# VikParuchuri/surya

Hardware: AMD Instinct MI355X
Metric: text-lines/sec recognised (whole node) (higher is better)
Workload: dtype bf16; 1 GPU; RecognitionPredictor device loop, 256 ragged 64x{128..512} crops/GPU, batch 256, max_tokens=48, REC-FULL synthetic weights (conditioned recipe, seed 0), tiles resident in HBM; parallelism=1 GPU, weights=conditioned

## Files before the change

surya_amd/csrc/common.h:

```cpp
#pragma once
#include <hip/hip_runtime.h>
#include <cstdlib>
#include <stdint.h>
#include <stdio.h>
#include <type_traits>

#include "../../include/surya_amd.h"

namespace sa {

typedef unsigned short bf16_t;
typedef __attribute__((ext_vector_type(4))) float f32x4;
typedef __attribute__((ext_vector_type(16))) float f32x16;
typedef __attribute__((ext_vector_type(8))) __bf16 bf16x8;
typedef unsigned int u32x4 __attribute__((ext_vector_type(4)));


#define SA_HIP(expr)                                                                                   \
    do {                                                                                               \
        hipError_t _e = (expr);                                                                        \
        if (_e != hipSuccess) {                                                                        \
            fprintf(stderr, "[surya_amd] %s:%d %s -> %s\n", __FILE__, __LINE__, #expr, hipGetErrorString(_e)); \
            return (int)_e;                                                                            \
        }                                                                                              \
// ... 163 lines not shown
    e8 = e + 127;
    return mx_pack4(ldexpf(v[0], -e), ldexpf(v[1], -e), ldexpf(v[2], -e), ldexpf(v[3], -e));
}

__device__ __forceinline__ float wave_sum(float v) {
#pragma unroll
    for (int o = 32; o > 0; o >>= 1) v += __shfl_xor(v, o, 64);
    return v;
}
__device__ __forceinline__ float wave_max(float v) {
#pragma unroll
    for (int o = 32; o > 0; o >>= 1) v = fmaxf(v, __shfl_xor(v, o, 64));
    return v;
}

__device__ __forceinline__ float silu_f(float x) { return x / (1.0f + __expf(-x)); }
template <typename TI>
__device__ __forceinline__ float silu_epi(float x) {
    if constexpr (sizeof(TI) == 2) return x * __builtin_amdgcn_rcpf(1.0f + __expf(-x));
    else return silu_f(x);
}
__device__ __forceinline__ float gelu_erf_f(float x) { return 0.5f * x * (1.0f + erff(x * 0.70710678118654752440f)); }
template <typename TI>
__device__ __forceinline__ float gelu_epi(float x) {
    if constexpr (std::is_same<TI, fp16_t>::value) {
        const float xr = Ty<fp16_t>::rnd(x);
        const float z = fabsf(xr) * 0.70710678118654752440f;
        const float t = __builtin_amdgcn_rcpf(fmaf(0.5f, z, 1.0f));
        float p = fmaf(t, 0.17087277f, -0.82215223f);
        p = fmaf(t, p, 1.48851587f);
        p = fmaf(t, p, -1.13520398f);
        p = fmaf(t, p, 0.27886807f);
        p = fmaf(t, p, -0.18628806f);
        p = fmaf(t, p, 0.09678418f);
        p = fmaf(t, p, 0.37409196f);
        p = fmaf(t, p, 1.00002368f);
        p = fmaf(t, p, -1.26551223f);
        const float e = t * __expf(fmaf(-z, z, p));
        return 0.5f * xr * (xr < 0.f ? e : 2.0f - e);
    } else if constexpr (sizeof(TI) == 2) {
        const float z = fabsf(x) * 0.70710678118654752440f;
        const float t = __builtin_amdgcn_rcpf(fmaf(0.3275911f, z, 1.0f));
        const float poly = t * fmaf(t, fmaf(t, fmaf(t, fmaf(t, 1.061405429f, -1.453152027f), 1.421413741f), -0.284496736f), 0.254829592f);
        const float erfc_abs = poly * __expf(-z * z);
        return 0.5f * x * (x < 0.f ? erfc_abs : 2.0f - erfc_abs);
    } else {
        return gelu_erf_f(x);
    }
}
__device__ __forceinline__ float gelu_tanh_f(float x) { return 0.5f * x * (1.0f + tanhf(0.7978845608028654f * (x + 0.044715f * x * x * x))); }
__device__ __forceinline__ float sigmoid_f(float x) { return 1.0f / (1.0f + __expf(-x)); }
__device__ __forceinline__ float hardswish_f(float x) {
    float t;
    asm("v_fma_f32 %0, %1, %2, 0.5 clamp" : "=v"(t) : "v"(x), "s"(1.0f / 6.0f));
    return x * t;
}
typedef float f32x2_hs __attribute__((ext_vector_type(2)));
__device__ __forceinline__ f32x2_hs hardswish_pk(f32x2_hs x) {
    f32x2_hs t;
    const f32x2_hs c = {1.0f / 6.0f, 1.0f / 6.0f};
    asm("v_pk_fma_f32 %0, %1, %2, 0.5 op_sel_hi:[1,0,0] clamp" : "=v"(t) : "v"(x), "s"(c));
    return x * t;
}

struct Tuning {
    int graph = 0;
    int split_target = 256;
    int split_min_kt = 4;
    int split_max = 8;
    int bigtile = 3;
    int bigtile_any = 0;
    int big_m_split = -1;
    int big_m_gateup = -1;
    int mx_big_m_split = -1;
    int mx_big_m_gateup = -1;
    int gateup_ring = 2;
    int dring = 1;
    int dring_min_kt = 0;
    int conv_persist = 3;
    int dwconv_pipe = 2;
    int conv_lean = 1;
    int bigtile_ratio_pct = 0;
    int bigtile_min_k = 0;
    int glds = 2;
    int dattn = 4;
    int rnorm = 2;
    int ghead = 2;
    int fuse_embed = 1;
    int kvprefetch = 0;
    int lmhead = 1;
    int dattn_db = 0;
    int lay_ln = 1;
    int det_head_blk = 1;
    int det_fuse = 1023;
    int det_up4 = 1;
    int fmb_chunk = 64;
    int persist = 1;
    int ocrerr_cls_only = 1;
};
inline Tuning& tuning() { static Tuning t; return t; }
inline int& tuning_epoch() { static int e = 0; return e; }

inline void poison_arena(void* p, size_t bytes) {
    static const bool on = [] { const char* e = getenv("SURYA_AMD_POISON"); return e && e[0] == '1'; }();
    if (on) { (void)hipMemset(p, 0xFF, bytes); (void)hipDeviceSynchronize(); }
}

struct AttrOnce {
    size_t granted[64] = {};
    template <typename F> void ensure(F kern, size_t lds) {
        int dev = 0;
        (void)hipGetDevice(&dev);
        size_t& g = granted[dev & 63];
        if (lds > g || g == 0) {
            (void)hipFuncSetAttribute(reinterpret_cast<const void*>(kern), hipFuncAttributeMaxDynamicSharedMemorySize, (int)lds);
            g = lds > g ? lds : g;
            if (g == 0) g = 1;
        }
    }
};

constexpr int SA_ALT_NONE = 0x7fffffff;
__device__ __forceinline__ bool alt_after(float v, int c, float pv, int pc) { return (v < pv) | ((v == pv) & (c > pc)); }
__device__ __forceinline__ bool alt_before(float v, int c, float bv, int bc) { return (v > bv) | ((v == bv) & (c < bc)); }
__device__ __forceinline__ float2 alt_next(const float2* cand, int n, float pv, int pc) {
    float cb = -INFINITY;
    int ci = SA_ALT_NONE;
    for (int k = 0; k < n; ++k) {
        const float v = cand[k].x;
        const int cc = __float_as_int(cand[k].y);
        const bool take = (v > -INFINITY) & alt_after(v, cc, pv, pc) & alt_before(v, cc, cb, ci);
        cb = take ? v : cb;
        ci = take ? cc : ci;
    }
    return make_float2(cb, __int_as_float(ci));
}

static inline int cdiv(int a, int b) { return (a + b - 1) / b; }
static inline long cdivl(long a, long b) { return (a + b - 1) / b; }

}
```

surya_amd/csrc/gemm.h:

```cpp
#pragma once
#include <algorithm>
#include <cstdlib>
#include <type_traits>

#include "common.h"
#include "fastdiv.h"

namespace sa {

enum GemmEpi { EPI_BIAS = 0, EPI_RESIDUAL = 1, EPI_GELU = 2, EPI_SWIGLU = 3, EPI_HARDSWISH = 4, EPI_RELU = 5, EPI_ARGMAX = 6, EPI_ROPE = 7,
               EPI_GEGLU = 8 ,
               EPI_ARGMAX_MASK = 9 ,
               EPI_TOPK = 10 ,
               EPI_FORCED = 11  };
constexpr bool epi_is_argmax(int epi) { return epi == EPI_ARGMAX || epi == EPI_ARGMAX_MASK || epi == EPI_TOPK || epi == EPI_FORCED; }
constexpr bool epi_is_masked(int epi) { return epi == EPI_ARGMAX_MASK || epi == EPI_TOPK; }

struct TokenMask {
    const uint32_t* table = nullptr;
    const int* slot_mask = nullptr;
    const int* row_slot = nullptr;
    int words = 0;
    __device__ __forceinline__ int id_of(int m, int M) const {
        const int gm = min(m, M - 1);
        return slot_mask[row_slot ? row_slot[gm] : gm];
    }
    __device__ __forceinline__ uint32_t word_of(int mid, int w) const {
        const uint32_t v = table[(long)max(mid, 0) * words + min(w, words - 1)];
        return mid < 0 ? 0xffffffffu : v;
    }
    __device__ __forceinline__ int id_or_none(int m, int M) const { return table ? id_of(m, M) : -1; }
    __device__ __forceinline__ uint32_t word_or_all(int mid, int w) const {
        return mid < 0 ? 0xffffffffu : table[(long)mid * words + min(w, words - 1)];
    }
};

struct ForcedCols {
    const int* table = nullptr;
    const int* cursor = nullptr;
    const int* row_slot = nullptr;
    int stride = 0;
    float* flogit = nullptr;
    __device__ __forceinline__ int col_of(int m, int M, int N) const {
        if (m >= M) return -1;
        const int slot = row_slot ? row_slot[m] : m;
        const int cur = cursor ? cursor[slot] : 0;
        const int c = table[(long)slot * stride + min(max(cur, 0), stride - 1)];
        return (cur >= 0 && cur < stride && c < N) ? c : -1;
    }
};

template <typename TI, typename TO>
struct GemmArgs {
    const TI* X; long ldx;
    const TI* W; long ldw;
    TO* C; long ldc;
    const TI* bias;
    const TO* R; long ldr;
    int M, N, K;
    int splitk = 1;
    float* part = nullptr;
    int swz_m = 0, swz_n = 0;
    int mgroup = 0;
    float4* amax = nullptr;
    mutable int bn_used = 0;
    TokenMask tmask;
    float2* alt = nullptr;
    ForcedCols forced;
    const float2* rope = nullptr;
    int rope_cols = 0, rope_D = 0;
    const TI* conv_in = nullptr;
    const TI* conv_zero = nullptr;
    int cH = 0, cW = 0, cCin = 0, cHo = 0, cWo = 0, cKW = 0, cStride = 0, cPad = 0, cTaps = 0;
    int conv_lean = 1;
    FastDiv fd_hw, fd_wo;
    unsigned cv_m1 = 0, cv_m2 = 0;
    int cv_rowskip = 0;
#ifndef SA_P8_TIMING
#define SA_P8_TIMING 0
#endif
#if SA_P8_TIMING
    long long* dbg = nullptr;
#endif
};

template <typename TI> struct Mfma;
template <> struct Mfma<bf16_t> {
    __device__ static __forceinline__ void run(f32x16& acc, const u32x4& w, const u32x4& x) { acc = H16<bf16_t>::mfma(w, x, acc); }
};
// ... 1407 lines not shown
#if SA_P8_TIMING
        ++dbg_tile;
#endif
        if (!have_next) return;
        tile_m = nt_m; tile_n = nt_n;
    }
#undef SP_STAMP
#undef SP_PHASE
#undef SP_VM
#undef SP_MMA
#undef SP_RW
#undef SP_RX
#undef SP_REQX
#undef SP_REQW
#undef SP_REQ
}
#undef SA_COMPUTE
#undef SA_COMPUTE_FULL
#undef SA_COMPUTE_LEAN
#undef SA_FRAGS
#undef SA_MFMAS

struct GemmProfiler {
    static constexpr int NCFG = 4, POOL = 8192;
    static constexpr int NCFG_ALL = 6;
    bool enabled = false;
    hipEvent_t ev[2 * POOL];
    bool have_events = false;
    int n = 0;
    int cfg_of[POOL];
    double flops_of[POOL], bytes_of[POOL], slab_of[POOL];
    void start() {
        if (!have_events) {
            for (int i = 0; i < 2 * POOL; ++i) (void)hipEventCreate(&ev[i]);
            have_events = true;
        }
        n = 0; enabled = true;
    }
};
inline GemmProfiler& gemm_profiler() { static GemmProfiler p; return p; }
inline int gemm_cfg_id(int BM, int BN) { return (BM >= 128 && BN >= 128) ? 0 : (BM == 256 ? 1 : 2); }

template <typename TI, typename TO, int BM, int BN, int WM, int WN, int EPI, bool SPLIT = false, int GLDS = 0, bool CONV = false, int WAUX = 0>
static inline int launch_gemm_cfg(const GemmArgs<TI, TO>& a, hipStream_t s) {
    int tiles = SPLIT ? cdiv(cdiv(a.N, BN) * a.splitk, 8) * 8 * cdiv(a.M, BM) : cdiv(a.M, BM) * cdiv(a.N, BN);
    a.bn_used = BN;
    GemmArgs<TI, TO> aa = a;
    if (!SPLIT && !a.mgroup && BM >= 128 && BN >= 128) {
        const int tm = cdiv(a.M, BM), tn = cdiv(a.N, BN);
        constexpr int GRP = ((BM + BN) * 128 * (GLDS > 2 && GLDS != 8 ? GLDS : 2) > 80 * 1024) ? 32 : 64;
        if (tm * tn >= 8 * GRP) {
            aa.swz_n = cdiv(tn, cdiv(tn, 8));
            aa.swz_m = std::max(1, GRP / aa.swz_n);
            tiles = cdiv(tm * tn, 8 * GRP) * 8 * GRP;
        }
    }
    if (!SPLIT && aa.mgroup) tiles = cdiv(cdiv(a.N, BN), 8) * 8 * cdiv(a.M, BM);
    constexpr size_t out_w = ((EPI == EPI_SWIGLU || EPI == EPI_GEGLU) && !SPLIT) ? BN / 2 : BN;
    constexpr size_t out_bytes = (size_t)BM * out_w * (SPLIT ? sizeof(float) : sizeof(TO));
    constexpr size_t stage_bytes = (size_t)(BM + BN) * 128 * (GLDS > 2 && GLDS != 8 ? GLDS : 2);
    constexpr bool argmax_direct = epi_is_argmax(EPI) && ((size_t)BM * BN * 4 > 160 * 1024);
    constexpr size_t lds = (argmax_direct || stage_bytes > out_bytes) ? stage_bytes : out_bytes;
    auto kern = gemm_nt_kernel<TI, TO, BM, BN, WM, WN, EPI, SPLIT, GLDS, CONV, WAUX>;
    static AttrOnce attr;
    attr.ensure(kern, lds);
    GemmProfiler& pf = gemm_profiler();
    const bool prof = pf.enabled && pf.n < GemmProfiler::POOL;
    if (prof) (void)hipEventRecord(pf.ev[2 * pf.n], s);
    hipLaunchKernelGGL(kern, dim3(tiles), dim3(64 * WM * WN), lds, s, aa);
    if (prof) {
        (void)hipEventRecord(pf.ev[2 * pf.n + 1], s);
        pf.cfg_of[pf.n] = CONV ? 3 : gemm_cfg_id(BM, BN);
        pf.flops_of[pf.n] = CONV ? 2.0 * a.M * a.N * a.cTaps * a.cCin : 2.0 * a.M * a.N * a.K;
        const double outn = (EPI == EPI_SWIGLU || EPI == EPI_GEGLU) ? a.N / 2 : (epi_is_argmax(EPI) ? 4.0 * cdiv(a.N, BN) : a.N);
        const double xelems = CONV ? (double)a.M / std::max(1, a.cHo * a.cWo) * a.cH * a.cW * a.cCin : (double)a.M * a.K;
        pf.bytes_of[pf.n] = (xelems + (double)a.N * a.K) * sizeof(TI) + (double)a.M * outn * (SPLIT ? sizeof(TI) : sizeof(TO)) +
                            (EPI == EPI_RESIDUAL ? (double)a.M * a.N * sizeof(TO) : 0.0);
        pf.slab_of[pf.n] = SPLIT ? (double)a.splitk * a.M * a.N * 4.0 : 0.0;
        ++pf.n;
    }
    return (int)hipGetLastError();
}

template <typename TI, typename TO, int EPI, int CONV = 0>
static inline int launch_gemm_persist(const GemmArgs<TI, TO>& a, hipStream_t s) {
    constexpr int BM = 256, BN = 256, GRP = 32;
    const int tm = cdiv(a.M, BM), tn = cdiv(a.N, BN);
    GemmArgs<TI, TO> aa = a;
    a.bn_used = BN;
    aa.swz_n = cdiv(tn, cdiv(tn, 8));
    aa.swz_m = std::max(1, GRP / aa.swz_n);
    const int padded = cdiv(tm * tn, 8 * GRP) * 8 * GRP;
    static int n_cu_of[64] = {};
    int dev = 0;
    (void)hipGetDevice(&dev);
    int& n_cu = n_cu_of[dev & 63];
    if (!n_cu) {
        if (hipDeviceGetAttribute(&n_cu, hipDeviceAttributeMultiprocessorCount, dev) != hipSuccess || n_cu <= 0) n_cu = 256;
        n_cu = (n_cu / 8) * 8;
    }
    const int grid = std::min(padded, n_cu);
    constexpr size_t lds = (size_t)2 * (BM + BN) * 128 + 8 * 4096;
    auto kern = gemm_nt_p8p_kernel<TI, TO, EPI, CONV>;
    static AttrOnce attr;
    attr.ensure(kern, lds);
    GemmProfiler& pf = gemm_profiler();
    const bool prof = pf.enabled && pf.n < GemmProfiler::POOL;
    if (prof) (void)hipEventRecord(pf.ev[2 * pf.n], s);
    hipLaunchKernelGGL(kern, dim3(grid), dim3(512), lds, s, aa);
    if (prof) {
        (void)hipEventRecord(pf.ev[2 * pf.n + 1], s);
        pf.cfg_of[pf.n] = CONV ? 3 : gemm_cfg_id(BM, BN);
        pf.flops_of[pf.n] = CONV ? 2.0 * a.M * a.N * a.cTaps * a.cCin : 2.0 * a.M * a.N * a.K;
        const double outn = (EPI == EPI_SWIGLU || EPI == EPI_GEGLU) ? a.N / 2 : a.N;
        const double xelems = CONV ? (double)a.M / std::max(1, a.cHo * a.cWo) * a.cH * a.cW * a.cCin : (double)a.M * a.K;
        pf.bytes_of[pf.n] = (xelems + (double)a.N * a.K) * sizeof(TI) + (double)a.M * outn * sizeof(TO) +
                            (EPI == EPI_RESIDUAL ? (double)a.M * a.N * sizeof(TO) : 0.0);
        pf.slab_of[pf.n] = 0.0;
        ++pf.n;
    }
    return (int)hipGetLastError();
}

}
#include "gemm_ring.h"
namespace sa {

static inline bool gemm_misaligned(const void* p, size_t bytes) { return (reinterpret_cast<uintptr_t>(p) & (bytes - 1)) != 0; }
template <typename TI, typename TO>
static inline bool gemm_operands_ok(const GemmArgs<TI, TO>& a, bool with_r) {
    constexpr long CI = 16 / (long)sizeof(TI), CO = 16 / (long)sizeof(TO);
    if (a.K <= 0 || a.ldx % CI != 0 || a.ldw % CI != 0 || a.ldc % CO != 0) return false;
    if (gemm_misaligned(a.X, 16) || gemm_misaligned(a.W, 16) || gemm_misaligned(a.C, 16) || gemm_misaligned(a.part, 16)) return false;
    if (gemm_misaligned(a.bias, 4 * sizeof(TI))) return false;
    if (with_r && (a.ldr % CO != 0 || gemm_misaligned(a.R, 16))) return false;
    return true;
}

template <typename TI, typename TO, int EPI>
static inline int launch_gemm(const GemmArgs<TI, TO>& a, hipStream_t s) {
    if (a.M <= 0 || a.N <= 0) return SA_OK;
    if (!gemm_operands_ok(a, EPI == EPI_RESIDUAL)) return SA_ERR_SHAPE;
    if constexpr (EPI == EPI_ROPE) {
        if (!a.rope || gemm_misaligned(a.rope, 16) || a.rope_D <= 0 || a.rope_D % 4 != 0 || a.rope_cols < 4 || a.rope_cols % 4 != 0) return SA_ERR_SHAPE;
    }
    {
        const int n_out = (EPI == EPI_SWIGLU || EPI == EPI_GEGLU) ? a.N / 2 : a.N;
        if (a.K % Ty<TI>::KE != 0 || a.N % 4 != 0 || n_out % (16 / (int)sizeof(TO)) != 0 || a.ldc % (16 / (int)sizeof(TO)) != 0)
            return SA_ERR_SHAPE;
    }
    if constexpr (EPI == EPI_ARGMAX_MASK) {
        if (!a.tmask.table || !a.tmask.slot_mask || a.tmask.words != cdiv(a.N, 32)) return SA_ERR_ARG;
    }
    if constexpr (EPI == EPI_TOPK) {
        if (!a.alt || (a.tmask.table && (!a.tmask.slot_mask || a.tmask.words != cdiv(a.N, 32)))) return SA_ERR_ARG;
    }
    if constexpr (EPI == EPI_FORCED) {
        if (!a.forced.table || !a.forced.flogit || a.forced.stride <= 0) return SA_ERR_ARG;
    }
    if (a.M <= 256) {
        if constexpr (epi_is_argmax(EPI)) {
            if (a.N >= 64 * 512 && tuning().lmhead && (a.K / Ty<TI>::KE) % 2 == 0 && a.N % 4 == 0) {
                if constexpr (sizeof(TI) == 2)
                    if (tuning().lmhead == 2) return launch_gemm_cfg<TI, TO, 256, 320, 4, 2, EPI, false, 2, false, 2>(a, s);
                return launch_gemm_cfg<TI, TO, 256, 320, 4, 2, EPI, false, 2>(a, s);
            }
            if (a.N >= 64 * 512) return launch_gemm_cfg<TI, TO, 128, 128, 2, 2, EPI, false, 2>(a, s);
            return launch_gemm_cfg<TI, TO, 64, 64, 2, 2, EPI, false, 2>(a, s);
        }
        if (a.M > 128) {
            if (a.N >= 64 * 512) return launch_gemm_cfg<TI, TO, 128, 128, 2, 2, EPI, false, 2>(a, s);
            if constexpr (EPI == EPI_SWIGLU && sizeof(TI) == 2 && sizeof(TO) == 2) {
                const int rc = launch_gateup_ring(a, s);
                if (rc >= 0) return rc;
            }
            if constexpr (EPI == EPI_SWIGLU && sizeof(TI) == 2) {
                if (tuning().gateup_ring == 3) return launch_gemm_cfg<TI, TO, 64, 64, 2, 2, EPI, false, 3>(a, s);
                if (tuning().gateup_ring == 4) return launch_gemm_cfg<TI, TO, 64, 64, 2, 2, EPI, false, 4>(a, s);
            }
            return launch_gemm_cfg<TI, TO, 64, 64, 2, 2, EPI, false, 2>(a, s);
        }
        if (a.M > 64) {
            if (a.N >= 64 * 128) return launch_gemm_cfg<TI, TO, 128, 64, 4, 1, EPI>(a, s);
            return launch_gemm_cfg<TI, TO, 128, 32, 4, 1, EPI>(a, s);
        }
        if (a.N >= 64 * 128) return launch_gemm_cfg<TI, TO, 64, 64, 2, 2, EPI>(a, s);
        return launch_gemm_cfg<TI, TO, 64, 32, 2, 1, EPI>(a, s);
    }
    if constexpr (epi_is_argmax(EPI)) {
        if (a.N >= 64 * 512 && tuning().lmhead && (a.K / Ty<TI>::KE) % 2 == 0 && a.N % 4 == 0) {
            GemmArgs<TI, TO> g = a;
            g.mgroup = 1;
            int rc;
            if constexpr (sizeof(TI) == 2) {
                if (tuning().lmhead == 2) { rc = launch_gemm_cfg<TI, TO, 256, 320, 4, 2, EPI, false, 2, false, 2>(g, s); a.bn_used = g.bn_used; return rc; }
            }
            rc = launch_gemm_cfg<TI, TO, 256, 320, 4, 2, EPI, false, 2>(g, s);
            a.bn_used = g.bn_used;
            return rc;
        }
    }
    if constexpr (EPI == EPI_SWIGLU && sizeof(TI) == 2 && sizeof(TO) == 2) {
        const int mode = tuning().big_m_gateup;
        const int rb = cdiv(a.M, 256), t256 = rb * cdiv(a.N, 256);
        const int pick = mode >= 0 ? mode : ((rb >= 4 && t256 >= 160 && t256 < 256) ? 2 : 0);
        if (pick && (a.K / Ty<TI>::KE) % 2 == 0 && a.K / Ty<TI>::KE >= 4 && a.N % 8 == 0) {
            if (pick == 1) return launch_gemm_persist<TI, TO, EPI>(a, s);
            return launch_gemm_cfg<TI, TO, 256, 256, 4, 2, EPI, false, 8>(a, s);
        }
    }
    if (a.N <= 64 && a.M >= 128 * 256) return launch_gemm_cfg<TI, TO, 128, 64, 4, 1, EPI>(a, s);
    const long big = (long)cdiv(a.M, 128) * cdiv(a.N, 128);
    const int glds = tuning().glds;
    if constexpr (sizeof(TO) == 2) {
        const int bigtile = tuning().bigtile;
        const long t256 = (long)cdiv(a.M, 256) * cdiv(a.N, 256);
        const double ratio256 = tuning().bigtile_ratio_pct > 0 ? tuning().bigtile_ratio_pct / 100.0
                                                                : ((bigtile == 3 && sizeof(TI) == 2) ? 1.4 : 1.17);
        const double cost256 = (double)cdivl(t256, 256) * 256 * 4 / ratio256, cost128 = (double)cdivl(big, 512) * 512;
        if (bigtile && a.K >= tuning().bigtile_min_k && ((t256 >= 256 && cost256 <= cost128) || tuning().bigtile_any)) {
            if constexpr (!epi_is_argmax(EPI)) {
                const int nk = a.K / Ty<TI>::KE;
                if constexpr (sizeof(TI) == 2)
                    if (tuning().persist && nk >= 4 && nk % 2 == 0 && a.N % 8 == 0) return launch_gemm_persist<TI, TO, EPI>(a, s);
            }
            if constexpr (sizeof(TI) == 2 && !epi_is_argmax(EPI)) {
                if (bigtile == 2 && (a.K / Ty<TI>::KE) % 2 == 0) return launch_gemm_cfg<TI, TO, 256, 256, 2, 2, EPI, false, 2>(a, s);
                if (bigtile == 3 && (a.K / Ty<TI>::KE) % 2 == 0) return launch_gemm_cfg<TI, TO, 256, 256, 4, 2, EPI, false, 8>(a, s);
            }
            return launch_gemm_cfg<TI, TO, 256, 256, 4, 2, EPI, false, 2>(a, s);
        }
    }
    if (big >= 256) {
        if (glds == 2) return launch_gemm_cfg<TI, TO, 128, 128, 2, 2, EPI, false, 2>(a, s);
        if (glds == 3) return launch_gemm_cfg<TI, TO, 128, 128, 2, 2, EPI, false, 3>(a, s);
        return launch_gemm_cfg<TI, TO, 128, 128, 2, 2, EPI>(a, s);
    }
    return launch_gemm_cfg<TI, TO, 64, 64, 2, 2, EPI>(a, s);
}

static inline int pick_splitk(int tiles_n, int nk) {
    const Tuning& t = tuning();
    const int tiles = tiles_n * 4;
    int s = (t.split_target + tiles / 2) / tiles;
    s = std::min(s, nk / std::max(1, t.split_min_kt));
    return std::max(1, std::min(s, std::min(t.split_max, 8)));
}

template <typename TI>
static inline int launch_gemm_splitk(GemmArgs<TI, TI>& a, hipStream_t s) {
    if (a.M <= 0 || a.N <= 0) return SA_OK;
    if (a.K % Ty<TI>::KE != 0 || a.N % 4 != 0 || !a.part) return SA_ERR_SHAPE;
    if (!gemm_operands_ok(a, false)) return SA_ERR_SHAPE;
    const int nk = a.K / Ty<TI>::KE;
    a.splitk = pick_splitk(cdiv(a.N, 64), nk);
    if constexpr (sizeof(TI) == 2) {
        const int mode = tuning().big_m_split;
        const int w128 = cdiv(a.M, 128) * cdiv(a.N, 128) * a.splitk, w12864 = cdiv(a.M, 128) * cdiv(a.N, 64) * a.splitk;
        const int pick = a.M <= 256 ? 0 : (mode >= 0 ? mode : (w128 >= 136 ? 2 : (w12864 <= 256 ? 3 : 0)));
        if (pick == 2) return launch_gemm_cfg<TI, TI, 128, 128, 2, 2, EPI_BIAS, true, 4>(a, s);
        if (pick == 3) return launch_gemm_cfg<TI, TI, 128, 64, 4, 1, EPI_BIAS, true, 4>(a, s);
    }
    if constexpr (sizeof(TI) == 2) {
        const int rc = launch_splitk_ring(a, s);
        if (rc >= 0) return rc;
    }
    return launch_gemm_cfg<TI, TI, 64, 64, 2, 2, EPI_BIAS, true, 4>(a, s);
}

}
```

surya_amd/csrc/rec_model.hip:

```cpp
#include "rec_engine.h"
#include "rec_ops.h"
#include "rec_prep.h"
#include "rec_rectify.h"
#include "rec_unroll.h"
#include "page_warp.h"
#include "rec_adjust.h"

namespace sa {

template <int D, int MAXG>
static int decode_attn_flash(const DecodeAttnArgs<bf16_t>& a, hipStream_t s) {
    const Tuning& t = tuning();
    if (t.dattn == 3) return decode_attn_as<decode_attn_flash_kernel<D, MAXG>>(a, decode_attn_flash_lds<D, MAXG>(), s, a.out8, a.sout, a.srows);
    if (t.dattn_db == 1 || (t.dattn_db == 0 && !t.graph && a.ctx_bound > 128 && a.rows * a.nkv <= 256))
        return decode_attn_as<decode_attn_flash2_kernel<D, MAXG, true>>(a, decode_attn_flash2_lds<D, MAXG, true>(), s, a.out8, a.sout, a.srows);
    return decode_attn_as<decode_attn_flash2_kernel<D, MAXG, false>>(a, decode_attn_flash2_lds<D, MAXG, false>(), s, a.out8, a.sout, a.srows);
}
template <typename T>
int launch_decode_attn(const DecodeAttnArgs<T>& a, hipStream_t s) {
    const int G = a.nq / a.nkv, d = a.d;
    if constexpr (std::is_same<T, bf16_t>::value) {
        if (d == 128 && G <= 5) return decode_attn_flash<128, 5>(a, s);
        if (d == 128 && G <= 8) return decode_attn_flash<128, 8>(a, s);
        if (d == 64 && G <= 8) return decode_attn_flash<64, 8>(a, s);
// ... 581 lines not shown
}

int surya_op_mx_quantize(const float* x, int rows, int K, uint8_t* q, uint8_t* scales, void* stream) {
    if (!x || !q || !scales || rows <= 0 || K <= 0 || K % 128) return SA_ERR_ARG;
    hipLaunchKernelGGL(mx_quantize_rows_kernel, dim3(rows), dim3(256), 0, (hipStream_t)stream, x, K, q, scales);
    return (int)hipGetLastError();
}

int surya_op_gemm_splitk_bf16(const void* X, long ldx, const void* W, long ldw, float* part, int M, int N, int K, int* splitk, void* stream) {
    if (!X || !W || !part || !splitk) return SA_ERR_ARG;
    GemmArgs<bf16_t, bf16_t> a{reinterpret_cast<const bf16_t*>(X), ldx, reinterpret_cast<const bf16_t*>(W), ldw, nullptr, 0, nullptr, nullptr, 0, M, N, K, 1, part};
    const int rc = launch_gemm_splitk<bf16_t>(a, (hipStream_t)stream);
    *splitk = a.splitk;
    return rc;
}

int surya_op_gemm_mx(int mode, const uint8_t* X, const uint8_t* SX, const uint8_t* W, const uint8_t* SW, int M, int N, int K,
                     float* C, int* splitk, uint8_t* q_out, uint8_t* sq_out, void* stream) {
    if (!X || !SX || !W || !SW) return SA_ERR_ARG;
    MxArgs a{X, (long)K, SX, W, (long)K, SW, M, N, K, (long)M, (long)N};
    hipStream_t s = (hipStream_t)stream;
    if (mode == 0) {
        if (!C) return SA_ERR_ARG;
        a.C = C; a.ldc = N;
        return launch_gemm_mx<MX_EPI_F32>(a, s);
    }
    if (mode == 1) {
        if (!C || !splitk) return SA_ERR_ARG;
        a.part = C;
        int rc = launch_gemm_mx_splitk(a, s);
        *splitk = a.splitk;
        return rc;
    }
    if (mode == 2) {
        if (!q_out || !sq_out) return SA_ERR_ARG;
        a.Q = q_out; a.ldq = N / 2; a.SQ = sq_out; a.sq_rows = M;
        return launch_gemm_mx<MX_EPI_SWIGLU>(a, s);
    }
    return SA_ERR_ARG;
}

int surya_rec_preprocess(const uint8_t* pages, const void* lines, int n_lines, uint8_t* mask_arena, float* mid_arena, float* tiles,
                         int patch_size, int merge_size, float pad_value, const float* mean, const float* std, int any_poly,
                         int max_stage1_width, int pixel_stride, void* stream) {
    if (!pages || !lines || !tiles || !mean || !std || n_lines < 0 || patch_size <= 0 || merge_size <= 0) return SA_ERR_ARG;
    if (pixel_stride != 3 && pixel_stride != 4) return SA_ERR_ARG;
    sa::prep::PrepArgs p;
    p.pages = pages; p.lines = reinterpret_cast<const sa::prep::LineDesc*>(lines); p.n_lines = n_lines;
    p.mask = mask_arena; p.mid = mid_arena; p.tiles = tiles; p.ps = patch_size; p.merge = merge_size; p.pad = pad_value;
    for (int i = 0; i < 3; ++i) { p.mean[i] = mean[i]; p.std[i] = std[i]; }
    p.max_mid_w = max_stage1_width;
    p.pix = pixel_stride;
    return sa::prep::prep_run(p, any_poly, max_stage1_width > 0, (hipStream_t)stream);
}

int surya_rec_rectify(const uint8_t* pages, const void* descs, int n, uint8_t* out, int pixel_stride, int max_w, int max_h, void* stream) {
    return sa::prep::rectify_run(pages, reinterpret_cast<const sa::prep::RectifyDesc*>(descs), n, out, pixel_stride, max_w, max_h,
                                 (hipStream_t)stream);
}

int surya_rec_unroll(const uint8_t* pages, const void* descs, int n, const double* tables, uint8_t* out, int pixel_stride, int max_w,
                     int max_h, void* stream) {
    return sa::prep::unroll_run(pages, reinterpret_cast<const sa::prep::UnrollDesc*>(descs), n, tables, out, pixel_stride, max_w, max_h,
                                (hipStream_t)stream);
}

int surya_warp_mesh(const uint8_t* pages, const void* descs, int n, const double* meshes, uint8_t* out, int pixel_stride, int max_w,
                    int max_h, void* stream) {
    return sa::prep::warp_mesh_run(pages, reinterpret_cast<const sa::pagewarp::MeshDesc*>(descs), n, meshes, out, pixel_stride, max_w, max_h,
                                   (hipStream_t)stream);
}

int surya_rec_adjust_contrast(const uint8_t* pages, const void* descs, int n, uint8_t* out, uint8_t* mask_arena, void* work, int32_t* lo_hi,
                              int pixel_stride, void* stream) {
    return sa::prep::adjust_run(pages, reinterpret_cast<const sa::adjust::AdjustDesc*>(descs), n, out, mask_arena, work, lo_hi, pixel_stride,
                                (hipStream_t)stream);
}

int surya_set_tuning(const char* key, int value) {
    if (!key) return SA_ERR_ARG;
    Tuning& t = tuning();
    struct { const char* k; int* v; } tab[] = {
        {"graph", &t.graph}, {"split_target", &t.split_target}, {"split_min_kt", &t.split_min_kt}, {"split_max", &t.split_max},
        {"bigtile", &t.bigtile}, {"bigtile_any", &t.bigtile_any}, {"conv_lean", &t.conv_lean}, {"conv_persist", &t.conv_persist}, {"dwconv_pipe", &t.dwconv_pipe}, {"bigtile_ratio_pct", &t.bigtile_ratio_pct}, {"gateup_ring", &t.gateup_ring}, {"dring", &t.dring}, {"dring_min_kt", &t.dring_min_kt}, {"big_m_split", &t.big_m_split}, {"big_m_gateup", &t.big_m_gateup}, {"mx_big_m_split", &t.mx_big_m_split}, {"mx_big_m_gateup", &t.mx_big_m_gateup}, {"glds", &t.glds}, {"bigtile_min_k", &t.bigtile_min_k}, {"dattn", &t.dattn}, {"rnorm", &t.rnorm},
        {"ghead", &t.ghead}, {"fuse_embed", &t.fuse_embed}, {"persist", &t.persist}, {"lmhead", &t.lmhead}, {"kvprefetch", &t.kvprefetch},
        {"dattn_db", &t.dattn_db}, {"lay_ln", &t.lay_ln}, {"det_head_blk", &t.det_head_blk}, {"det_fuse", &t.det_fuse}, {"det_up4", &t.det_up4}, {"fmb_chunk", &t.fmb_chunk}, {"ocrerr_cls_only", &t.ocrerr_cls_only}};
    for (auto& e : tab)
        if (!strcmp(e.k, key)) {
            if (*e.v != value) ++tuning_epoch();
            *e.v = value;
            return SA_OK;
        }
    return SA_ERR_ARG;
}

int surya_gemm_ring_status(int reset) {
    const int a = sa::ring_error(reset != 0), b = sa::rec_f16_ring_error(reset != 0);
    return a ? a : b;
}

int surya_prof_enable(int on) {
    GemmProfiler& pf = gemm_profiler();
    if (on) pf.start(); else pf.enabled = false;
    return SA_OK;
}

__global__ void prof_null_kernel() {}

int surya_prof_event_overhead(void* stream, double* ms) {
    if (!ms) return SA_ERR_ARG;
    hipStream_t s = (hipStream_t)stream;
    constexpr int N = 201;
    hipEvent_t ev[2 * N];
    for (auto& e : ev) SA_HIP(hipEventCreate(&e));
    for (int i = 0; i < 32; ++i) hipLaunchKernelGGL(prof_null_kernel, dim3(1), dim3(64), 0, s);
    for (int i = 0; i < N; ++i) {
        SA_HIP(hipEventRecord(ev[2 * i], s));
        hipLaunchKernelGGL(prof_null_kernel, dim3(1), dim3(64), 0, s);
        SA_HIP(hipEventRecord(ev[2 * i + 1], s));
    }
    SA_HIP(hipStreamSynchronize(s));
    std::vector<float> t(N);
    for (int i = 0; i < N; ++i) SA_HIP(hipEventElapsedTime(&t[i], ev[2 * i], ev[2 * i + 1]));
    for (auto& e : ev) (void)hipEventDestroy(e);
    std::sort(t.begin(), t.end());
    *ms = t[N / 2];
    return SA_OK;
}

int surya_prof_read2(int max_cfg, int* launches, double* ms, double* flops, double* bytes, double* slab_bytes) {
    GemmProfiler& pf = gemm_profiler();
    if (!launches || !ms || !flops || !bytes || max_cfg < GemmProfiler::NCFG) return SA_ERR_ARG;
    SA_HIP(hipDeviceSynchronize());
    const int ncfg = std::min(max_cfg, (int)GemmProfiler::NCFG_ALL);
    for (int c = 0; c < ncfg; ++c) { launches[c] = 0; ms[c] = flops[c] = bytes[c] = 0.0; if (slab_bytes) slab_bytes[c] = 0.0; }
    for (int i = 0; i < pf.n; ++i) {
        const int c = pf.cfg_of[i];
        if (c >= ncfg) continue;
        float t = 0.f;
        SA_HIP(hipEventElapsedTime(&t, pf.ev[2 * i], pf.ev[2 * i + 1]));
        launches[c]++; ms[c] += t; flops[c] += pf.flops_of[i]; bytes[c] += pf.bytes_of[i];
        if (slab_bytes) slab_bytes[c] += pf.slab_of[i];
    }
    pf.n = 0;
    return SA_OK;
}

int surya_prof_read(int max_cfg, int* launches, double* ms, double* flops, double* bytes) {
    return surya_prof_read2(max_cfg, launches, ms, flops, bytes, nullptr);
}

int surya_op_rmsnorm(int dtype, const void* x, long ldx, const void* w, void* y, long ldy, int rows, int C, float eps,
                     void* stream) {
    if (!x || !w || !y || rows <= 0) return SA_ERR_ARG;
    hipStream_t s = (hipStream_t)stream;
    if (dtype == SA_DTYPE_F32) return sa::launch_rmsnorm<float>((const float*)x, ldx, (const float*)w, (float*)y, ldy, nullptr, rows, C, eps, s);
    if (dtype == SA_DTYPE_BF16) return sa::launch_rmsnorm<bf16_t>((const bf16_t*)x, ldx, (const bf16_t*)w, (bf16_t*)y, ldy, nullptr, rows, C, eps, s);
    return SA_ERR_UNSUPPORTED;
}

static int rec_dispatch(int dtype, int op, const void* a, void* stream) {
    hipStream_t s = (hipStream_t)stream;
    if (dtype == SA_DTYPE_F32) return sa::rec_op_any<float>(op, a, s);
    if (dtype == SA_DTYPE_BF16) return sa::rec_op_any<bf16_t>(op, a, s);
    if (dtype == SA_DTYPE_F16) return sa::op_rec_f16(op, a, s);
    return SA_ERR_UNSUPPORTED;
}
// ... 101 lines not shown
```

Measured before the change: 3204 lines/s.

## Peel GEMM rows into a big-tile head launch and a smaller-tile tail

Adds a cost-model planner that splits a GEMM's M dimension. The head is a whole number of 256-row blocks sized to fill full CU waves with the persistent 256x256 kernel. The remaining rows are sent back through the normal dispatcher with peeling disabled, so they go to the 128-tile or small-M path. The aim is to cut wave-quantization waste on tall GEMMs whose tile count does not evenly fill the CUs. The cost is an extra kernel launch per split GEMM, and the split choice depends on a heuristic cost model that may be miscalibrated.

Measured after the change: 3216 lines/s, median of 2. Within noise of the previous version (+0.4%).

```diff
diff --git a/surya_amd/csrc/common.h b/surya_amd/csrc/common.h
--- a/surya_amd/csrc/common.h
+++ b/surya_amd/csrc/common.h
@@ -269,6 +269,7 @@
     int conv_lean = 1;
     int bigtile_ratio_pct = 0;
     int bigtile_min_k = 0;
+    int mpeel = 1;
     int glds = 2;
     int dattn = 4;
     int rnorm = 2;
diff --git a/surya_amd/csrc/gemm.h b/surya_amd/csrc/gemm.h
--- a/surya_amd/csrc/gemm.h
+++ b/surya_amd/csrc/gemm.h
@@ -5,6 +5,7 @@
 
 #include "common.h"
 #include "fastdiv.h"
+#include "gemm_plan_core.h"
 
 namespace sa {
 
@@ -1578,6 +1579,18 @@
     return (int)hipGetLastError();
 }
 
+static inline int gemm_n_cu() {
+    static int n_cu_of[64] = {};
+    int dev = 0;
+    (void)hipGetDevice(&dev);
+    int& n_cu = n_cu_of[dev & 63];
+    if (!n_cu) {
+        if (hipDeviceGetAttribute(&n_cu, hipDeviceAttributeMultiprocessorCount, dev) != hipSuccess || n_cu <= 0) n_cu = 256;
+        n_cu = (n_cu / 8) * 8;
+    }
+    return n_cu;
+}
+
 template <typename TI, typename TO, int EPI, int CONV = 0>
 static inline int launch_gemm_persist(const GemmArgs<TI, TO>& a, hipStream_t s) {
     constexpr int BM = 256, BN = 256, GRP = 32;
@@ -1587,15 +1600,7 @@
     aa.swz_n = cdiv(tn, cdiv(tn, 8));
     aa.swz_m = std::max(1, GRP / aa.swz_n);
     const int padded = cdiv(tm * tn, 8 * GRP) * 8 * GRP;
-    static int n_cu_of[64] = {};
-    int dev = 0;
-    (void)hipGetDevice(&dev);
-    int& n_cu = n_cu_of[dev & 63];
-    if (!n_cu) {
-        if (hipDeviceGetAttribute(&n_cu, hipDeviceAttributeMultiprocessorCount, dev) != hipSuccess || n_cu <= 0) n_cu = 256;
-        n_cu = (n_cu / 8) * 8;
-    }
-    const int grid = std::min(padded, n_cu);
+    const int grid = std::min(padded, gemm_n_cu());
     constexpr size_t lds = (size_t)2 * (BM + BN) * 128 + 8 * 4096;
     auto kern = gemm_nt_p8p_kernel<TI, TO, EPI, CONV>;
     static AttrOnce attr;
@@ -1634,7 +1639,22 @@
 }
 
 template <typename TI, typename TO, int EPI>
-static inline int launch_gemm(const GemmArgs<TI, TO>& a, hipStream_t s) {
+static inline int launch_gemm_big(const GemmArgs<TI, TO>& a, hipStream_t s) {
+    const int bigtile = tuning().bigtile;
+    if constexpr (!epi_is_argmax(EPI)) {
+        const int nk = a.K / Ty<TI>::KE;
+        if constexpr (sizeof(TI) == 2)
+            if (tuning().persist && nk >= 4 && nk % 2 == 0 && a.N % 8 == 0) return launch_gemm_persist<TI, TO, EPI>(a, s);
+    }
+    if constexpr (sizeof(TI) == 2 && !epi_is_argmax(EPI)) {
+        if (bigtile == 2 && (a.K / Ty<TI>::KE) % 2 == 0) return launch_gemm_cfg<TI, TO, 256, 256, 2, 2, EPI, false, 2>(a, s);
+        if (bigtile == 3 && (a.K / Ty<TI>::KE) % 2 == 0) return launch_gemm_cfg<TI, TO, 256, 256, 4, 2, EPI, false, 8>(a, s);
+    }
+    return launch_gemm_cfg<TI, TO, 256, 256, 4, 2, EPI, false, 2>(a, s);
+}
+
+template <typename TI, typename TO, int EPI>
+static inline int launch_gemm(const GemmArgs<TI, TO>& a, hipStream_t s, bool peel = true) {
     if (a.M <= 0 || a.N <= 0) return SA_OK;
     if (!gemm_operands_ok(a, EPI == EPI_RESIDUAL)) return SA_ERR_SHAPE;
     if constexpr (EPI == EPI_ROPE) {
@@ -1714,18 +1734,26 @@
         const double ratio256 = tuning().bigtile_ratio_pct > 0 ? tuning().bigtile_ratio_pct / 100.0
                                                                 : ((bigtile == 3 && sizeof(TI) == 2) ? 1.4 : 1.17);
         const double cost256 = (double)cdivl(t256, 256) * 256 * 4 / ratio256, cost128 = (double)cdivl(big, 512) * 512;
-        if (bigtile && a.K >= tuning().bigtile_min_k && ((t256 >= 256 && cost256 <= cost128) || tuning().bigtile_any)) {
-            if constexpr (!epi_is_argmax(EPI)) {
-                const int nk = a.K / Ty<TI>::KE;
-                if constexpr (sizeof(TI) == 2)
-                    if (tuning().persist && nk >= 4 && nk % 2 == 0 && a.N % 8 == 0) return launch_gemm_persist<TI, TO, EPI>(a, s);
-            }
-            if constexpr (sizeof(TI) == 2 && !epi_is_argmax(EPI)) {
-                if (bigtile == 2 && (a.K / Ty<TI>::KE) % 2 == 0) return launch_gemm_cfg<TI, TO, 256, 256, 2, 2, EPI, false, 2>(a, s);
-                if (bigtile == 3 && (a.K / Ty<TI>::KE) % 2 == 0) return launch_gemm_cfg<TI, TO, 256, 256, 4, 2, EPI, false, 8>(a, s);
-            }
-            return launch_gemm_cfg<TI, TO, 256, 256, 4, 2, EPI, false, 2>(a, s);
-        }
+        if constexpr (sizeof(TI) == 2 && !epi_is_argmax(EPI)) {
+            const int mpeel = tuning().mpeel;
+            if (peel && mpeel && bigtile && a.K >= tuning().bigtile_min_k) {
+                const gemmplan::Plan pl = gemmplan::plan_rows(a.M, a.N, a.K, gemm_n_cu(), ratio256, tuning().bigtile_any != 0, mpeel == 2);
+                if (pl.rows_big > 0 && pl.rows_big < a.M) {
+                    GemmArgs<TI, TO> head = a, rest = a;
+                    head.M = pl.rows_big;
+                    rest.M = a.M - pl.rows_big;
+                    rest.X = a.X + (size_t)pl.rows_big * a.ldx;
+                    rest.C = a.C + (size_t)pl.rows_big * a.ldc;
+                    if (a.R) rest.R = a.R + (size_t)pl.rows_big * a.ldr;
+                    if constexpr (EPI == EPI_ROPE) rest.rope = a.rope + (size_t)pl.rows_big * (a.rope_D / 2);
+                    const int rc = launch_gemm_big<TI, TO, EPI>(head, s);
+                    if (rc) return rc;
+                    return launch_gemm<TI, TO, EPI>(rest, s, false);
+                }
+            }
+        }
+        if (bigtile && a.K >= tuning().bigtile_min_k && ((t256 >= 256 && cost256 <= cost128) || tuning().bigtile_any))
+            return launch_gemm_big<TI, TO, EPI>(a, s);
     }
     if (big >= 256) {
         if (glds == 2) return launch_gemm_cfg<TI, TO, 128, 128, 2, 2, EPI, false, 2>(a, s);
diff --git a/surya_amd/csrc/gemm_plan_core.h b/surya_amd/csrc/gemm_plan_core.h
--- /dev/null
+++ b/surya_amd/csrc/gemm_plan_core.h
@@ -0,0 +1,80 @@
+#pragma once
+
+namespace sa {
+namespace gemmplan {
+
+enum Path { PATH_NONE = 0, PATH_BIG = 1, PATH_T128 = 2, PATH_SMALL = 3 };
+
+constexpr double SMALL_FIXED = 0.22;
+constexpr double SMALL_PER_KT = 0.8;
+
+struct Plan {
+    int rows_big = 0;
+    int rest_path = PATH_NONE;
+    int whole_path = PATH_NONE;
+    int rounds_big = 0;
+    double cost = 0.0;
+    double cost_whole = 0.0;
+};
+
+inline long plan_cdiv(long a, long b) { return (a + b - 1) / b; }
+
+inline double cost_big(long rows, int N, int n_cu, double ratio) {
+    const long t = plan_cdiv(rows, 256) * plan_cdiv(N, 256);
+    return (double)(plan_cdiv(t, n_cu) * n_cu) * 4.0 / ratio;
+}
+inline double cost_t128(long rows, int N, int n_cu) {
+    const long t = plan_cdiv(rows, 128) * plan_cdiv(N, 128);
+    return (double)(plan_cdiv(t, 2L * n_cu) * 2L * n_cu);
+}
+inline long small_workgroups(int rows, int N) {
+    if (rows > 128) return N >= 64 * 512 ? plan_cdiv(rows, 128) * plan_cdiv(N, 128) : plan_cdiv(rows, 64) * plan_cdiv(N, 64);
+    if (rows > 64) return plan_cdiv(N, N >= 64 * 128 ? 64 : 32);
+    return plan_cdiv(N, N >= 64 * 128 ? 64 : 32);
+}
+inline double cost_small(int rows, int N, int K, int n_cu) {
+    const double nk = K >= 64 ? K / 64.0 : 1.0;
+    return (double)plan_cdiv(small_workgroups(rows, N), 2L * n_cu) * n_cu * (SMALL_FIXED / nk + SMALL_PER_KT);
+}
+inline double cost_alone(long rows, int N, int K, int n_cu, double ratio, bool force_big, int* path) {
+    if (rows <= 256) { *path = PATH_SMALL; return cost_small((int)rows, N, K, n_cu); }
+    const long t256 = plan_cdiv(rows, 256) * plan_cdiv(N, 256);
+    const double cb = cost_big(rows, N, n_cu, ratio), c1 = cost_t128(rows, N, n_cu);
+    if (force_big || (t256 >= n_cu && cb <= c1)) { *path = PATH_BIG; return cb; }
+    *path = PATH_T128;
+    return c1;
+}
+
+inline Plan plan_rows(int M, int N, int K, int n_cu, double ratio, bool force_big = false, bool force_split = false) {
+    Plan p;
+    if (M <= 256 || N <= 0 || K <= 0 || n_cu <= 0 || !(ratio > 0.0)) return p;
+    p.cost_whole = cost_alone(M, N, K, n_cu, ratio, force_big, &p.whole_path);
+    p.cost = p.cost_whole;
+    const long tiles_n = plan_cdiv(N, 256), full = M / 256;
+    if (force_split) {
+        p.rows_big = 256 * ((M - 1) / 256);
+        p.rounds_big = (int)plan_cdiv((long)(p.rows_big / 256) * tiles_n, n_cu);
+        p.cost = cost_big(p.rows_big, N, n_cu, ratio) + cost_alone(M - p.rows_big, N, K, n_cu, ratio, force_big, &p.rest_path);
+        return p;
+    }
+    const long k_max = plan_cdiv(plan_cdiv(M, 256) * tiles_n, n_cu);
+    long last = 0;
+    for (long k = 1; k <= k_max; ++k) {
+        long blocks = k * n_cu / tiles_n;
+        if (blocks > full) blocks = full;
+        if (blocks <= 0 || blocks == last || blocks * 256 >= M) continue;
+        last = blocks;
+        int path;
+        const double c = cost_big(blocks * 256, N, n_cu, ratio) + cost_alone(M - blocks * 256, N, K, n_cu, ratio, force_big, &path);
+        if (c < p.cost) {
+            p.cost = c;
+            p.rows_big = (int)(blocks * 256);
+            p.rest_path = path;
+            p.rounds_big = (int)plan_cdiv(blocks * tiles_n, n_cu);
+        }
+    }
+    return p;
+}
+
+}
+}
diff --git a/surya_amd/csrc/rec_model.hip b/surya_amd/csrc/rec_model.hip
--- a/surya_amd/csrc/rec_model.hip
+++ b/surya_amd/csrc/rec_model.hip
@@ -687,7 +687,7 @@
     Tuning& t = tuning();
     struct { const char* k; int* v; } tab[] = {
         {"graph", &t.graph}, {"split_target", &t.split_target}, {"split_min_kt", &t.split_min_kt}, {"split_max", &t.split_max},
-        {"bigtile", &t.bigtile}, {"bigtile_any", &t.bigtile_any}, {"conv_lean", &t.conv_lean}, {"conv_persist", &t.conv_persist}, {"dwconv_pipe", &t.dwconv_pipe}, {"bigtile_ratio_pct", &t.bigtile_ratio_pct}, {"gateup_ring", &t.gateup_ring}, {"dring", &t.dring}, {"dring_min_kt", &t.dring_min_kt}, {"big_m_split", &t.big_m_split}, {"big_m_gateup", &t.big_m_gateup}, {"mx_big_m_split", &t.mx_big_m_split}, {"mx_big_m_gateup", &t.mx_big_m_gateup}, {"glds", &t.glds}, {"bigtile_min_k", &t.bigtile_min_k}, {"dattn", &t.dattn}, {"rnorm", &t.rnorm},
+        {"bigtile", &t.bigtile}, {"bigtile_any", &t.bigtile_any}, {"mpeel", &t.mpeel},{"conv_lean", &t.conv_lean}, {"conv_persist", &t.conv_persist}, {"dwconv_pipe", &t.dwconv_pipe}, {"bigtile_ratio_pct", &t.bigtile_ratio_pct}, {"gateup_ring", &t.gateup_ring}, {"dring", &t.dring}, {"dring_min_kt", &t.dring_min_kt}, {"big_m_split", &t.big_m_split}, {"big_m_gateup", &t.big_m_gateup}, {"mx_big_m_split", &t.mx_big_m_split}, {"mx_big_m_gateup", &t.mx_big_m_gateup}, {"glds", &t.glds}, {"bigtile_min_k", &t.bigtile_min_k}, {"dattn", &t.dattn}, {"rnorm", &t.rnorm},
         {"ghead", &t.ghead}, {"fuse_embed", &t.fuse_embed}, {"persist", &t.persist}, {"lmhead", &t.lmhead}, {"kvprefetch", &t.kvprefetch},
         {"dattn_db", &t.dattn_db}, {"lay_ln", &t.lay_ln}, {"det_head_blk", &t.det_head_blk}, {"det_fuse", &t.det_fuse}, {"det_up4", &t.det_up4}, {"fmb_chunk", &t.fmb_chunk}, {"ocrerr_cls_only", &t.ocrerr_cls_only}};
     for (auto& e : tab)
```
